# christopher-beckham/gan-heightmaps

Measured on AMD Instinct MI355X. Metric: 512px heightmap+texture train images/sec, higher is better.
Workload: dtype bf16x3; 1 GPU; test1_nobn_bilin_both joint DCGAN+pix2pix train step (train_mode=both), 512x512, batch 4 per GPU, RMSprop lr 1e-4, LSGAN+100*L1; fp32 by operand splitting on the bf16 matrix cores (3 exact bf16 pieces per operand, 6 products, fp32 accumulation); global_batch=4, in_shp=512, parallelism=dp1, hip_graph=False, issue=recorded, streams=3

## Files before the change

### gan_heightmaps_amd/_lib.py

```python
import ctypes as C
import os

_HERE = os.path.dirname(os.path.abspath(__file__))
LIB_PATH = os.path.join(_HERE, "libghm.so")


class GhmError(RuntimeError):
    pass


class ConvDesc(C.Structure):
    _fields_ = [("N", C.c_int32), ("C", C.c_int32), ("H", C.c_int32), ("W", C.c_int32),
                ("K", C.c_int32), ("Ho", C.c_int32), ("Wo", C.c_int32),
                ("kh", C.c_int32), ("kw", C.c_int32), ("stride", C.c_int32), ("pad", C.c_int32),
                ("x_nstride", C.c_int64), ("y_nstride", C.c_int64)]


class RenderParams(C.Structure):
    _fields_ = [("pos", C.c_float * 3), ("yaw", C.c_float), ("pitch", C.c_float), ("fov", C.c_float),
                ("Hi", C.c_int32), ("Wi", C.c_int32),
                ("height_scale", C.c_float), ("step", C.c_float), ("max_dist", C.c_float),
                ("sun_azimuth", C.c_float), ("sun_elevation", C.c_float), ("shadows", C.c_int32),
                ("softness", C.c_float), ("ambient", C.c_float), ("haze", C.c_float),
                ("horizon", C.c_float * 3), ("zenith", C.c_float * 3), ("accel", C.c_int32), ("out_u8", C.c_int32)]
# ... 111 lines not shown
    "ghm_maxpool2_fwd": [_p, _p, _p, _i32, _i32, _i32, _i32],
    "ghm_maxpool2_bwd": [_p, _p, _p, _p, _p, _i32, _i32, _i32, _i32, _i32, _f],
    "ghm_avgpool_fwd": [_p, _p, _p, _i32, _i32, _i32, _i32, _i32],
    "ghm_avgpool_bwd": [_p, _p, _p, _i32, _i32, _i32, _i32, _i32],
    "ghm_dropout": [_p, _p, _i64, _p, _i64, _i32, _i32, _i32, _f, C.c_uint32, _p],
    "ghm_counter_tick": [_p, _p],
    "ghm_transpose_weights_batched": [_p, _p, _i32, _i32],
    "ghm_upconv_collapse_weights": [_p, _p, _p, _p, _p, _i32, _i32],
    "ghm_upconv_collapse_batched": [_p, _p, _i32, _i32],
    "ghm_upconv_expand_batched": [_p, _p, _i32, _i32, _i32],
    "ghm_blconv_frame_sizes": [_i32, _i32, _i32, _i32, _i32, C.POINTER(_i64), C.POINTER(_i64)],
    "ghm_blconv_frame_fwd": [_p, _p, _i64, _p, _p, _i64, _i32, _i32, _i32, _i32, _i32, _p],
    "ghm_blconv_frame_gather": [_p, _p, _i64, _i32, _i32, _i32, _i32, _i32, _p],
    "ghm_blconv_frame_dgrad": [_p, _p, _p, _p, _i64, _i32, _i32, _i32, _i32, _i32],
    "ghm_blconv_frame_wgrad": [_p, _p, _p, _p, _i32, _i32, _i32, _i32, _i32],
    "ghm_blconv_fwd_split": [_p, _D, _p, _i64, _i64, _p, _p, _p, _i32],
    "ghm_blconv_dgrad_split": [_p, _D, _p, _i64, _i64, _p, _p, _i32, _i32],
    "ghm_blconv_wgrad_split": [_p, _D, _p, _i64, _i64, _p, _i64, _i64, _p, _p, _i32, _i32],
    "ghm_upconv_expand_wgrad": [_p, _p, _p, _i32, _i32, _i32],
    "ghm_pp_to_hi": [_p, _p, _p, _i64, _i32, _i32, _i32, _i32],
    "ghm_hi_to_pp": [_p, _p, _i64, _p, _i32, _i32, _i32, _i32],
    "ghm_upsample_nearest2_fwd": [_p, _p, _i64, _p, _i32, _i32, _i32, _i32],
    "ghm_upsample_nearest2_bwd": [_p, _p, _p, _i64, _i32, _i32, _i32, _i32, _i32],
    "ghm_upsample_bilinear2_fwd": [_p, _p, _i64, _p, _i32, _i32, _i32, _i32],
    "ghm_upsample_bilinear2_bwd": [_p, _p, _p, _i64, _i32, _i32, _i32, _i32, _i32],
    "ghm_copy_view": [_p, _p, _i64, _p, _i64, _i32, _i32, _i32, _i32],
    "ghm_scale_samples": [_p, _p, _i64, _i32, _i32, _i32, _p, _i64, _p, _i64],
    "ghm_axpby": [_p, _f, _p, _f, _p, _i64],
    "ghm_image_batch": [_p, _p, _i32, _i32, _i32, _i32, _p, _i32, _p, _i64],
    "ghm_texture_gather": [_p, _p, _i32, _i32, _i32, _i32, _i32, _i32, _i32, _i32, _i32, _i32, _i32, _i32, _i32, _p, _i64],
# ... 25 lines not shown
    "ghm_comm_destroy": [_p],
    "ghm_comm_count": [_p, C.POINTER(_i32)],
    "ghm_allreduce_sum": [_p, _p, _i64],
    "ghm_allreduce_sum_bf16": [_p, _p, _i64, _p],
    "ghm_allreduce_max": [_p, _p, _i64],
    "ghm_reduce_scatter_sum": [_p, _p, _i64],
    "ghm_all_gather": [_p, _p, _i64],
    "ghm_conv2d_variant": [_D, _i32, C.c_char_p, _i32],
}
_SPECIAL = {"ghm_last_error": ([], C.c_char_p), "ghm_bn_workspace": ([_i32], C.c_size_t),
            "ghm_dgrad_t_supported": ([_D], C.c_int), "ghm_lp_supported": ([_D, _i32, _i32], C.c_int),
            "ghm_conv2d_pool_supported": ([_D, _i32, _i32], C.c_int),
            "ghm_dgrad_dact_supported": ([_D, _i32], C.c_int),
            "ghm_blconv_supported": ([_i32, _i32, _i32, _i32, _i32], C.c_int),
            "ghm_blconv_split_supported": ([_D, _i32], C.c_int),
            "ghm_lp_q_direct": ([_D, _i32, _i32], C.c_int),
            "ghm_conv_bn_fused_supported": ([_D, _i32], C.c_int),
            "ghm_conv_bn_fused_supported_f32": ([_D], C.c_int),
            "ghm_lp_wgrad_q_supported": ([_D, _i32], C.c_int),
            "ghm_split_supported": ([_D, _i32], C.c_int),
            "ghm_conv2d_wgrad_pooled_split_supported": ([_D], C.c_int),
            "ghm_split_pool_supported": ([_D, _i32], C.c_int),
            "ghm_split_q_direct": ([_D, _i32], C.c_int),
            "ghm_split_dgrad_dact_supported": ([_D], C.c_int),
            "ghm_render_maxmip_elems": ([_i32, _i32], C.c_int64)}

_lib = None


def load():
# ... 55 lines not shown
```

### gan_heightmaps_amd/csrc/conv_bilinear.hip

```cpp
#include <stdlib.h>
#include <string.h>

#include "common.h"

namespace {

typedef float f32x16 __attribute__((ext_vector_type(16)));

__device__ __forceinline__ int bl_job_line(int job) { return job == 0 ? 0 : (job < 3 ? 1 : (job == 3 ? 2 : 3)); }
__device__ __forceinline__ int bl_job_tap(int job, int t) {
    const int fixed = (job == 0 || job == 3) ? 0 : ((job == 1 || job == 4) ? 2 : 1);
    return job < 3 ? fixed * 3 + t : t * 3 + fixed;
}

struct BlGeo {
    int N, C, K, n1, n2, LP;
};

__global__ __launch_bounds__(256) void bl_lines_kernel(const float* __restrict__ x, long xs, BlGeo g, float* __restrict__ FL,
                                                       float* __restrict__ FLt) {
    const long idx = (long)blockIdx.x * 256 + threadIdx.x;
    const long total = (long)g.N * 4 * g.C * g.LP;
    if (idx >= total) return;
    const int ai = (int)(idx % g.LP);
// ... 66 lines not shown
#pragma unroll 4
    for (int c0 = c_lo + 2 * wave; c0 < c_hi; c0 += 8) {
        const int c = c0 + kg;
        const float* w = wp + (long)c * 9 * g.K + k;
        const float* f = fl + (long)c * g.LP;
        const float a0 = w[(long)t0 * g.K], a1 = w[(long)t1 * g.K], a2 = w[(long)t2 * g.K];
        const float b0 = f[0], b1 = f[1], b2 = f[2];
        acc = bl_mfma(a0, b0, acc);
        acc = bl_mfma(a1, b1, acc);
        acc = bl_mfma(a2, b2, acc);
    }
    float* dst = DL + ((((long)sp * 6 + job) * g.N + n) * g.K + blockIdx.x * 32) * g.LP + blockIdx.y * 32;
    bl_reduce_store(acc, dst, g.LP, 1, smem, 32, 32);
}

__global__ __launch_bounds__(256) void bl_wt_kernel(const float* __restrict__ wp, int C, int K, float* __restrict__ wT) {
    const long idx = (long)blockIdx.x * 256 + threadIdx.x;
    if (idx >= (long)9 * K * C) return;
    const int c = (int)(idx % C);
    const long r = idx / C;
    const int k = (int)(r % K), tap = (int)(r / K);
    wT[idx] = wp[((long)c * 9 + tap) * K + k];
}

__global__ __launch_bounds__(256) void bl_gemm_dgrad_kernel(const float* __restrict__ wT, const float* __restrict__ DYL, BlGeo g,
                                                            int splits, float* __restrict__ dFL, int wp_direct) {
    __shared__ float smem[4 * 32 * 33];
    const int lane = threadIdx.x & 63, wave = threadIdx.x >> 6, li = lane & 31, kg = lane >> 5;
    int z = blockIdx.z;
    const int n = z % g.N;
// ... 17 lines not shown
        const float* w1 = wp_direct ? wT + ((long)c * 9 + bl_job_tap(job, 1)) * g.K : wT + bl_job_tap(job, 1) * KC + c;
        const float* w2 = wp_direct ? wT + ((long)c * 9 + bl_job_tap(job, 2)) * g.K : wT + bl_job_tap(job, 2) * KC + c;
#pragma unroll 4
        for (int k0 = k_lo + 2 * wave; k0 < k_hi; k0 += 8) {
            const int k = k0 + kg;
            const float a0 = w0[k * ks], a1 = w1[k * ks], a2 = w2[k * ks];
            const float* d = dy + (long)k * LD;
            const float b0 = d[0], b1 = d[-1], b2 = d[-2];
            acc = bl_mfma(a0, b0, acc);
            acc = bl_mfma(a1, b1, acc);
            acc = bl_mfma(a2, b2, acc);
        }
    }
    float* dst = dFL + ((((long)sp * g.N + n) * 4 + line) * g.C + blockIdx.x * 32) * g.LP + blockIdx.y * 32;
    bl_reduce_store(acc, dst, g.LP, 1, smem, 32, 32);
}

__global__ __launch_bounds__(256) void bl_gemm_wgrad_kernel(const float* __restrict__ DYLt, const float* __restrict__ FLt, BlGeo g,
                                                            int splits, float* __restrict__ dWp, float* __restrict__ direct) {
    __shared__ float smem[4 * 32 * 33];
    const int lane = threadIdx.x & 63, wave = threadIdx.x >> 6, li = lane & 31, kg = lane >> 5;
    const int tap = blockIdx.z % 9, sp = blockIdx.z / 9;
    const int A = tap / 3, B = tap % 3;
    const int k = blockIdx.x * 32 + li, c = blockIdx.y * 32 + li;
    const int LD = g.LP + 32;
    const int rowjob = A == 0 ? 0 : (A == 2 ? 1 : 2), coljob = B == 0 ? 3 : (B == 2 ? 4 : 5);
    const int rowline = A == 0 ? 0 : 1, colline = B == 0 ? 2 : 3;
    f32x16 acc;
#pragma unroll
    for (int e = 0; e < 16; ++e) acc[e] = 0.f;
// ... 140 lines not shown
    *fl_floats = 2 * ((int64_t)N * 4 * C * LP + 64);
    *dyl_floats = 2 * ((int64_t)6 * N * K * (LP + 32));
    return 0;
}

int ghm_blconv_supported(int32_t N, int32_t C, int32_t K, int32_t n1, int32_t n2) { return bl_ok(N, C, K, n1, n2) ? 1 : 0; }

static int bl_splits(long contraction, long tiles, int num_cu) {
    int s = (int)((4L * num_cu + tiles - 1) / tiles);
    const int smax = (int)(contraction / 256);
    if (s > smax) s = smax;
    if (s > 32) s = 32;
    return s < 1 ? 1 : s;
}

int ghm_blconv_frame_fwd(ghm_ctx* ctx, const float* x, int64_t x_nstride, const float* wp, float* y, int64_t y_nstride, int32_t N,
                         int32_t C, int32_t K, int32_t n1, int32_t n2, float* FL) {
    GHM_CHECK(bl_ok(N, C, K, n1, n2), "ghm_blconv_frame_fwd: geometry not served");
    const BlGeo g{N, C, K, n1, n2, bl_lp(n1, n2)};
    hipLaunchKernelGGL(bl_lines_kernel, dim3(ceil_div((long)N * 4 * C * g.LP, 256)), dim3(256), 0, ctx->stream, x, (long)x_nstride, g, FL,
                       FL + ((long)N * 4 * C * g.LP + 64));
    GHM_LAUNCH_CHECK();
    const int used = (2 * (n1 > n2 ? n1 : n2) + 31) / 32;
    const int splits = bl_splits(3L * C, (long)(K / 32) * used * 6 * N, ctx->num_cu);
    void* ws;
    if (ghm_scratch(ctx, (size_t)splits * 6 * N * K * g.LP * 4, &ws)) return -1;
    hipLaunchKernelGGL(bl_gemm_fwd_kernel, dim3(K / 32, used, splits * 6 * N), dim3(256), 0, ctx->stream, wp, (const float*)FL, g, splits,
                       (float*)ws);
    GHM_LAUNCH_CHECK();
    const long nb = 3L * 2 * n2 + 3L * (2 * n1 - 3);
    hipLaunchKernelGGL(bl_scatter_fwd_kernel, dim3(ceil_div((long)N * K * nb, 256)), dim3(256), 0, ctx->stream, (const float*)ws, g, splits,
                       y, (long)y_nstride);
    GHM_LAUNCH_CHECK();
    return 0;
}

int ghm_blconv_frame_gather(ghm_ctx* ctx, const float* dy, int64_t dy_nstride, int32_t N, int32_t C, int32_t K, int32_t n1, int32_t n2,
                            float* DYL) {
    GHM_CHECK(bl_ok(N, C, K, n1, n2), "ghm_blconv_frame_gather: geometry not served");
    const BlGeo g{N, C, K, n1, n2, bl_lp(n1, n2)};
    hipLaunchKernelGGL(bl_gather_dy_kernel, dim3(ceil_div((long)6 * N * K * (g.LP + 32), 256)), dim3(256), 0, ctx->stream, dy,
                       (long)dy_nstride, g, DYL, DYL + (long)6 * N * K * (g.LP + 32));
    GHM_LAUNCH_CHECK();
    return 0;
}

int ghm_blconv_frame_dgrad(ghm_ctx* ctx, const float* DYL, const float* wp, float* dx, int64_t dx_nstride, int32_t N, int32_t C,
                           int32_t K, int32_t n1, int32_t n2) {
    GHM_CHECK(bl_ok(N, C, K, n1, n2), "ghm_blconv_frame_dgrad: geometry not served");
    const BlGeo g{N, C, K, n1, n2, bl_lp(n1, n2)};
    const int used = (2 * (n1 > n2 ? n1 : n2) + 2 + 31) / 32;
    const int splits = bl_splits(6L * K, (long)(C / 32) * used * 4 * N, ctx->num_cu);
    void* ws;
    const size_t part_bytes = (size_t)splits * N * 4 * C * g.LP * 4;
    if (ghm_scratch(ctx, part_bytes + (size_t)9 * K * C * 4, &ws)) return -1;
    float* const wT = (float*)((char*)ws + part_bytes);
    const int direct = GHM_OPT("GHM_BLCONV_NO_WT") ? 1 : 0;
    if (!direct) {
        hipLaunchKernelGGL(bl_wt_kernel, dim3(ceil_div((long)9 * K * C, 256)), dim3(256), 0, ctx->stream, wp, C, K, wT);
        GHM_LAUNCH_CHECK();
    }
    hipLaunchKernelGGL(bl_gemm_dgrad_kernel, dim3(C / 32, used, splits * 4 * N), dim3(256), 0, ctx->stream,
                       direct ? wp : (const float*)wT, DYL, g, splits, (float*)ws, direct);
    GHM_LAUNCH_CHECK();
    const long nb = (long)(n1 >= 2 ? 2 : 1) * n2 + (long)(n2 >= 2 ? 2 : 1) * (n1 > 2 ? n1 - 2 : 0);
    hipLaunchKernelGGL(bl_fold_kernel, dim3(ceil_div((long)N * C * nb, 256)), dim3(256), 0, ctx->stream, (const float*)ws, g, splits, dx,
                       (long)dx_nstride);
// ... 13 lines not shown
                           DYL + (long)6 * N * K * (g.LP + 32), FL + ((long)N * 4 * C * g.LP + 64), g, 1, (float*)nullptr, dwp);
        GHM_LAUNCH_CHECK();
        return 0;
    }
    void* ws;
    if (ghm_scratch(ctx, (size_t)splits * 9 * C * K * 4, &ws)) return -1;
    hipLaunchKernelGGL(bl_gemm_wgrad_kernel, dim3(K / 32, C / 32, splits * 9), dim3(256), 0, ctx->stream,
                       DYL + (long)6 * N * K * (g.LP + 32), FL + ((long)N * 4 * C * g.LP + 64), g, splits, (float*)ws, (float*)nullptr);
    GHM_LAUNCH_CHECK();
    hipLaunchKernelGGL(bl_wgrad_add_kernel, dim3(ceil_div((long)C * 9 * K, 256)), dim3(256), 0, ctx->stream, (const float*)ws, C, K, splits,
                       dwp);
    GHM_LAUNCH_CHECK();
    return 0;
}

}
```

### gan_heightmaps_amd/csrc/elementwise.hip

```cpp
#include "common.h"

namespace {

struct View {
    int N, C, HW;
};

template <int VEC>
__device__ __forceinline__ bool decode(const View v, long& n, long& c, long& i) {
    const long per_row = v.HW / VEC;
    const long idx = (long)blockIdx.x * blockDim.x + threadIdx.x;
    const long total = (long)v.N * v.C * per_row;
    if (idx >= total) return false;
    const long row = idx / per_row;
    i = (idx - row * per_row) * VEC;
    n = row / v.C;
    c = row - n * v.C;
    return true;
}

inline bool aligned16(const void* p) { return ((uintptr_t)p & 15) == 0; }

inline int grid_for(const View v, int vec) { return ceil_div((long)v.N * v.C * (v.HW / vec), 256); }

// ... 745 lines not shown
    float v = 0.f;
#pragma unroll
    for (int pq = 0; pq < 4; ++pq) {
        const int rs = upconv_group(pq >> 1, a) * 3 + upconv_group(pq & 1, b);
        v += dwpc[(((long)c * 9 + rs) * 4 + pq) * K + k];
    }
    dwp5[i] = accumulate ? dwp5[i] + v : v;
}

struct CollapseItem {
    const float* wp5;
    const float* bias;
    float* wpc;
    float* bias4;
    int C, K, block_begin, mode;
};

__device__ __forceinline__ float blconv_coef(int p, int r, int a) {
    if (p == 0) return r == 1 ? (a == 1 ? 1.f : 0.5f) : ((r == 0 && a == 0) || (r == 2 && a == 2) ? 0.5f : 0.f);
    return r == 0 ? 0.f : (a == 1 ? 0.5f : ((r == 1 && a == 0) || (r == 2 && a == 2) ? 1.f : 0.f));
}

__global__ __launch_bounds__(256) void upconv_collapse_batched_kernel(const CollapseItem* __restrict__ items, int n) {
    int li = 0;
    for (int i = 1; i < n; ++i)
        if ((int)blockIdx.x >= items[i].block_begin) li = i;
    const CollapseItem it = items[li];
    const long total = (long)it.C * 36 * it.K;
    const long i = (long)(blockIdx.x - it.block_begin) * 256 + threadIdx.x;
    if (i < total) {
        const int K = it.K;
        const int k = (int)(i % K);
        long t = i / K;
        const int pq = (int)(t % 4); t /= 4;
        const int rs = (int)(t % 9);
        const int c = (int)(t / 9);
        const int p = pq >> 1, q = pq & 1, r = rs / 3, s_ = rs % 3;
        float v = 0.f;
        if (it.mode == 1) {
            for (int a = 0; a < 3; ++a)
                for (int b = 0; b < 3; ++b) {
                    const float cf = blconv_coef(p, r, a) * blconv_coef(q, s_, b);
                    if (cf != 0.f) v += cf * it.wp5[((long)c * 9 + a * 3 + b) * K + k];
                }
// ... 762 lines not shown
```

### gan_heightmaps_amd/device.py

```python
import ctypes as C

import numpy as np

from . import _lib
from ._lib import ConvDesc, call

ACT_CODES = {'linear': 0, 'relu': 1, 'lrelu': 2, 'sigmoid': 3, 'tanh': 4}
DTYPE_CODES = {'f32': 0, 'bf16': 1, 'f16': 2}
SPLIT = 'bf16x3'
DTYPE_CODES[SPLIT] = 3
SPLIT2 = 'bf16x2'
DTYPE_CODES[SPLIT2] = 4
SPLITS = {SPLIT: 3, SPLIT2: 2}


def device_count():
    n = C.c_int32(0)
    call("ghm_device_count", C.byref(n))
    return n.value


class DevTensor:
    __slots__ = ("dev", "ptr", "shape", "nstride", "base")

# ... 376 lines not shown
        call("ghm_conv2d_fwd", self.h, C.byref(d), _vp(x), _vp(wp), _vp(bias), _vp(y), ACT_CODES[act], alpha,
             int(accumulate))

    def conv2d_dgrad(self, d, dy, wp, dx, bias=None, act='linear', alpha=0.0, accumulate=False):
        call("ghm_conv2d_dgrad", self.h, C.byref(d), _vp(dy), _vp(wp), _vp(bias), _vp(dx), ACT_CODES[act], alpha,
             int(accumulate))

    def dgrad_t_supported(self, d):
        return bool(_lib.load().ghm_dgrad_t_supported(C.byref(d)))

    def transpose_weights(self, d, wp, wpT):
        call("ghm_conv2d_transpose_weights", self.h, C.byref(d), _vp(wp), _vp(wpT))

    def collapse_table(self, items):
        rec = np.zeros(len(items), dtype=[('wp5', '<u8'), ('bias', '<u8'), ('wpc', '<u8'), ('b4', '<u8'), ('C', '<i4'),
                                          ('K', '<i4'), ('b0', '<i4'), ('pad', '<i4')])
        b0 = 0
        for i, (w5, b, wpc, b4, Cc, K, *mode) in enumerate(items):
            rec[i] = (w5.ptr, b.ptr if b is not None else 0, wpc.ptr, b4.ptr if b4 is not None else 0, Cc, K, b0, mode[0] if mode else 0)
            b0 += (36 * Cc * K + 4 * K + 255) // 256
        ptr = self.dev.alloc(max(rec.nbytes, 40))
        self.dev.h2d(ptr, rec.view(np.uint8))
        return ptr, len(items), b0

    def upconv_collapse_batched(self, table):
        ptr, n, blocks = table
        call("ghm_upconv_collapse_batched", self.h, C.c_void_p(ptr), n, blocks)

    def expand_table(self, items):
        rec = np.zeros(len(items), dtype=[('dwpc', '<u8'), ('dwp5', '<u8'), ('C', '<i4'), ('K', '<i4'), ('b0', '<i4'),
                                          ('pad', '<i4')])
        b0 = 0
        for i, (dwpc, dwp5, Cc, K, *mode) in enumerate(items):
            rec[i] = (dwpc.ptr, dwp5.ptr, Cc, K, b0, mode[0] if mode else 0)
            b0 += (25 * Cc * K + 255) // 256
        ptr = self.dev.alloc(max(rec.nbytes, 32))
# ... 11 lines not shown
        a, b = C.c_int64(), C.c_int64()
        call("ghm_blconv_frame_sizes", int(N), int(Cc), int(K), int(n1), int(n2), C.byref(a), C.byref(b))
        return a.value, b.value

    def blconv_frame_fwd(self, x, wp, y_pp, K, FL):
        call("ghm_blconv_frame_fwd", self.h, _vp(x), x.nstride, _vp(wp), _vp(y_pp), y_pp.nstride, x.N, x.Cc, int(K), x.H, x.W, _vp(FL))

    def blconv_frame_gather(self, dy_pp, Cc, K, DYL):
        call("ghm_blconv_frame_gather", self.h, _vp(dy_pp), dy_pp.nstride, dy_pp.N, int(Cc), int(K), dy_pp.H, dy_pp.W, _vp(DYL))

    def blconv_frame_dgrad(self, DYL, wp, dx, K):
        call("ghm_blconv_frame_dgrad", self.h, _vp(DYL), _vp(wp), _vp(dx), dx.nstride, dx.N, dx.Cc, int(K), dx.H, dx.W)

    def blconv_frame_wgrad(self, DYL, FL, dwp, N, Cc, K, n1, n2):
        call("ghm_blconv_frame_wgrad", self.h, _vp(DYL), _vp(FL), _vp(dwp), int(N), int(Cc), int(K), int(n1), int(n2))

    def blconv_split_supported(self, d, kind, dtype):
        return dtype in SPLITS and bool(_lib.load().ghm_blconv_split_supported(C.byref(d), int(kind)))

    def blconv_fwd_split(self, d, xq, wq, bias, y, dtype):
        call("ghm_blconv_fwd_split", self.h, C.byref(d), C.c_void_p(xq.ptr), xq.nstride, xq.pstride, _vp(wq), _vp(bias), _vp(y),
             SPLITS[dtype])

    def blconv_dgrad_split(self, d, dyq, wqT, dx, dtype, accumulate=False):
        call("ghm_blconv_dgrad_split", self.h, C.byref(d), C.c_void_p(dyq.ptr), dyq.nstride, dyq.pstride, _vp(wqT), _vp(dx),
             int(accumulate), SPLITS[dtype])

    def blconv_wgrad_split(self, d, xq, dyq, dwp, ws, dtype, accumulate=False):
        call("ghm_blconv_wgrad_split", self.h, C.byref(d), C.c_void_p(xq.ptr), xq.nstride, xq.pstride, C.c_void_p(dyq.ptr),
             dyq.nstride, dyq.pstride, _vp(dwp), _vp(ws), int(accumulate), SPLITS[dtype])
# ... 602 lines not shown
```

### gan_heightmaps_amd/engine.py

```python
import os

import numpy as np

from . import layers as L
from .architectures.layers import BilinearUpsample2DLayer
from .device import SPLITS, DevTensor, QTensor, conv_desc, pack_conv_w, unpack_conv_w
from .nonlinearities import linear

ALIGN = 64
FWD, DGRAD, WGRAD, DGRAD_T = 0, 1, 2, 3


def _align(n):
    return (n + ALIGN - 1) // ALIGN * ALIGN


class ParamStore:

    def __init__(self, dev, params, pad_to=1):
        self.dev = dev
        self.params = list(params)
        nt = ns = 0
        for p in self.params:
            n = int(np.prod(p.shape))
# ... 256 lines not shown

class NetPlan:

    def __init__(self, dev, ops, out_layer, batch, store, inputs=None, out_tensor=None, name="net", side=None,
                 bn_groups=1, rng_seed=0, rng_counter=None, dtype='f32'):
        self.dev, self.ops, self.batch, self.store, self.name = dev, ops, batch, store, name
        self.side = side
        assert dtype in ('f32', 'bf16', 'f16') or dtype in SPLITS, dtype
        self.dtype = dtype
        self.bn_groups = bn_groups
        nodes, of = _build_ir(out_layer)
        self.out_node = _rewrite(of[id(out_layer)], dtype)
        self.order = _toposort(self.out_node)
        self.node_of_layer = of
        self.input_nodes = [n for n in self.order if n.op == 'input']
        self._shapes()
        self._fuse_convpool()
        self._place(inputs or {}, out_tensor)
        self.use_q = self.dtype != 'f32' and os.environ.get("GHM_NO_Q") is None and hasattr(ops, 'q_pack')
        self.q_epi = self.use_q
        for n in self.order:
            n.outq = None
        if self.use_q:
            self._place_q()
        self._scratch = {}
        self._collapse_tab = None
        self._last_grads = {}
        self.bn_ws = None
        cmax = max([n.shape[1] for n in self.order if n.op == 'bn'] + [0])
        if cmax:
# ... 131 lines not shown
                    n.aux['mean_g'] = [n.aux['mean'], self.dev.empty((1, C, 1, 1))]
                    n.aux['inv_g'] = [n.aux['inv'], self.dev.empty((1, C, 1, 1))]
            if n.op == 'convpool':
                n.aux['mask'] = self.dev.alloc(int(np.prod(n.shape)))
            if n.op == 'upconv':
                C, K = n.inputs[0].shape[1], n.shape[1]
                for name in ('wpc', 'wpcT', 'dwpc'):
                    n.aux[name] = self.dev.empty((1, C * 9 * 4 * K, 1, 1))
                n.aux['b4'] = self.dev.empty((1, 4 * K, 1, 1))
                if n.attrs.get('mode') == 1:
                    xs = n.inputs[0].shape
                    if not self.ops.blconv_supported(xs[0], C, K, xs[2], xs[3]):
                        raise NotImplementedError("bilinear up-sample convolution %r: geometry not served by the library" % (n,))
                    nfl, ndyl = self.ops.blconv_frame_sizes(xs[0], C, K, xs[2], xs[3])
                    n.aux['fl'], n.aux['dyl'] = self.dev.empty((1, nfl, 1, 1)), self.dev.empty((1, ndyl, 1, 1))

    def _place_q(self):
        need = []
        for n in self.order:
            if n.op in ('conv', 'convpool'):
                d = self._desc(n, n.inputs[0].out, self._full(n))
            elif n.op == 'upconv':
                d = self._upconv_desc(n, n.inputs[0].out)
            else:
                continue
            if self._lp(d, FWD) and n.inputs[0].shape[1] % 8 == 0 and self._q_viewable(n.inputs[0]):
                need.append(n.inputs[0])

        def get_outq(n):
            if n.outq is not None:
# ... 151 lines not shown
        if b > self._wgrad_ws_bytes:
            if self.wgrad_ws is not None:
                self.dev.free(self.wgrad_ws)
            self.wgrad_ws = self.dev.alloc(b)
            self._wgrad_ws_bytes = b

    def emit_forward(self, prog, deterministic=False, update_running=True, lp_done=None):
        ops, st = self.ops, self.store
        if self.dropout_nodes and not deterministic:
            prog.append(("rng_tick", lambda c=self.rng_counter: ops.counter_tick(c)))
        ups = [n for n in self.order if n.op == 'upconv']
        if ups:
            if self._collapse_tab is None:
                self._collapse_tab = ops.collapse_table(
                    [(st.value(n.layer.W), st.value(n.layer.b), n.aux['wpc'], n.aux['b4'], n.inputs[0].shape[1], n.shape[1],
                      n.attrs.get('mode', 0)) for n in ups])
            prog.append(("collapse_w", lambda t=self._collapse_tab: ops.upconv_collapse_batched(t)))
        if self._lp_table is not None:
            prog.append(("lp_pack", lambda t=self._lp_table: ops.lp_pack_batched(t, self.dtype)))
        ctx = _ForwardCtx(prog, deterministic, update_running, lp_done)
        for n in self.order:
            if id(n) in ctx.fused_bn:
                continue
            lower = getattr(self, '_fwd_' + n.op, None)
            if lower is None:
                raise NotImplementedError(n.op)
            q_direct = lower(ctx, n)
            if n.outq is not None and not q_direct:
                self._q_pack(prog, n.out, n.outq)

    def _q_pack(self, prog, t, q):
# ... 165 lines not shown
        w5 = st.value(n.layer.W)
        wpc, b4, K = n.aux['wpc'], n.aux['b4'], n.shape[1]
        bl = n.attrs.get('mode') == 1
        label = ('blconv' if bl else 'upconv') + "_fwd"
        y4 = y.reshape((x.N, 4 * K, x.H, x.W))
        wq = None
        if self._lp(d, FWD):
            wq = self._lp_pack_entry(prog, d, wpc, ('c', id(n.layer.W)), False, None)
        if wq is not None and xq is not None and self._bl_skip(n, d, FWD) and a == linear:
            prog.append((label, lambda: ops.blconv_fwd_split(d, xq, wq, b4, y4, self.dtype), bl_meta(conv_meta(ops, d, FWD, self.dtype))))
        else:
            prog.append(self._conv_fwd_entry(label, d, x, xq, wpc, wq, b4, y4, None, a))
        if bl:
            if a != linear:
                raise NotImplementedError("bilinear up-sample convolution with its own nonlinearity")
            prog.append(("blconv_frame_fwd", lambda fl=n.aux['fl']: ops.blconv_frame_fwd(x, w5, y4, K, fl)))
        return False

    def _fwd_pp_to_hi(self, ctx, n):
        ops, x, y, yq = self.ops, n.inputs[0].out, n.out, n.outq
        if id(n) in ctx.fused_hi:
            return self.q_epi
        if yq is not None and self.q_epi and y.nstride % 2 == 0:
            y32 = y if self._fp32_needed(n) else None
            ctx.prog.append(("pp_to_hi", lambda: ops.pp_to_hi_q(x, y32, yq)))
            return True
        ctx.prog.append(("pp_to_hi", lambda: ops.pp_to_hi(x, y)))
        return False

    def _fwd_dropout(self, ctx, n):
        ops, x, y = self.ops, n.inputs[0].out, n.out
# ... 453 lines not shown
            if G4q is not None and plan._bl_skip(n, d, DGRAD):
                prog.append((label, lambda: ops.blconv_dgrad_split(d, G4q, wqT, gi, plan.dtype, acc),
                             bl_meta(conv_meta(ops, d, DGRAD_T, dt))))
            elif G4q is not None:
                prog.append((label, lambda: ops.conv2d_dgrad_lp_q(d, G4q, wqT, gi, None, plan.dtype, None, 'linear', 0.0, acc),
                             conv_meta(ops, d, DGRAD_T, dt)))
            else:
                prog.append((label, lambda: ops.conv2d_dgrad_lp(d, G4, wqT, gi, plan.dtype, None, 'linear', 0.0, acc),
                             conv_meta(ops, d, DGRAD_T, dt)))
        elif C > 4 and ops.dgrad_t_supported(d):
            self.transpose_once(('c', id(l.W)), d, wpc, wpcT)
            prog.append((label, lambda: ops.conv2d_dgrad_t(d, G4, wpcT, gi, None, 'linear', 0.0, acc), conv_meta(ops, d, DGRAD_T)))
        else:
            prog.append((label, lambda: ops.conv2d_dgrad(d, G4, wpc, gi, None, 'linear', 0.0, acc), conv_meta(ops, d, DGRAD)))
        if bl:
            prog.append(("blconv_frame_dgrad", lambda dyl=n.aux['dyl'], w3=self.st.value(l.W): ops.blconv_frame_dgrad(dyl, w3, gi, K)))

    def bwd_dropout(self, n, G, xin, x, y, need_dx):
        if need_dx:
            gi, acc = self.target(xin)
            if acc or self.nslice is not None:
                raise NotImplementedError("DropoutLayer input with several consumers / sample slices")
            ops = self.ops
            self.prog.append(("dropout_bwd", lambda p=n.attrs['p'], k=n.aux['key'], c=self.plan.rng_counter: ops.dropout(G, gi, p, k, c)))
            self.mark_written(xin)

    def bwd_pp_to_hi(self, n, G, xin, x, y, need_dx):
        if need_dx and self.nslice is None and self.plan._bn_hi(xin) and G.nstride % 2 == 0:
            self.grads[id(xin)] = G
            self.hi_grads.add(id(xin))
            self.mark_written(xin)
# ... 189 lines not shown
```

### include/ghm.h

```cpp
#ifndef GHM_H
#define GHM_H

#include <stddef.h>
#include <stdint.h>

#ifdef __cplusplus
extern "C" {
#endif

typedef struct ghm_ctx ghm_ctx;
typedef struct ghm_graph ghm_graph;
typedef struct ghm_step ghm_step;

enum { GHM_DTYPE_F32 = 0, GHM_DTYPE_BF16 = 1, GHM_DTYPE_F16 = 2 };

enum { GHM_ACT_LINEAR = 0, GHM_ACT_RELU = 1, GHM_ACT_LRELU = 2, GHM_ACT_SIGMOID = 3, GHM_ACT_TANH = 4 };

typedef struct {
    int32_t N;
    int32_t C, H, W;
    int32_t K, Ho, Wo;
    int32_t kh, kw, stride, pad;
    int64_t x_nstride;
    int64_t y_nstride;
// ... 192 lines not shown
int ghm_counter_tick(ghm_ctx* ctx, void* counter);
int ghm_upconv_collapse_weights(ghm_ctx* ctx, const float* wp5, const float* bias, float* wpc, float* bias4, int32_t C, int32_t K);
int ghm_upconv_collapse_batched(ghm_ctx* ctx, const void* table, int32_t n_items, int32_t total_blocks);
int ghm_upconv_expand_wgrad(ghm_ctx* ctx, const float* dwpc, float* dwp5, int32_t C, int32_t K, int32_t accumulate);
int ghm_upconv_expand_batched(ghm_ctx* ctx, const void* table, int32_t n_items, int32_t total_blocks, int32_t accumulate);
int ghm_blconv_supported(int32_t N, int32_t C, int32_t K, int32_t n1, int32_t n2);
int ghm_blconv_frame_sizes(int32_t N, int32_t C, int32_t K, int32_t n1, int32_t n2, int64_t* fl_floats, int64_t* dyl_floats);
int ghm_blconv_frame_fwd(ghm_ctx* ctx, const float* x, int64_t x_nstride, const float* wp, float* y_pp, int64_t y_nstride, int32_t N,
                         int32_t C, int32_t K, int32_t n1, int32_t n2, float* FL);
int ghm_blconv_frame_gather(ghm_ctx* ctx, const float* dy_pp, int64_t dy_nstride, int32_t N, int32_t C, int32_t K, int32_t n1,
                            int32_t n2, float* DYL);
int ghm_blconv_frame_dgrad(ghm_ctx* ctx, const float* DYL, const float* wp, float* dx, int64_t dx_nstride, int32_t N, int32_t C,
                           int32_t K, int32_t n1, int32_t n2);
int ghm_blconv_frame_wgrad(ghm_ctx* ctx, const float* DYL, const float* FL, float* dwp, int32_t N, int32_t C, int32_t K, int32_t n1,
                           int32_t n2);
int ghm_blconv_split_supported(const ghm_conv_desc* d, int32_t kind);
int ghm_blconv_fwd_split(ghm_ctx* ctx, const ghm_conv_desc* d, const void* xq, int64_t xq_nstride, int64_t xq_pstride, const void* wq,
                         const float* bias, float* y, int32_t pieces);
int ghm_blconv_dgrad_split(ghm_ctx* ctx, const ghm_conv_desc* d, const void* dyq, int64_t dyq_nstride, int64_t dyq_pstride,
                           const void* wqT, float* dx, int32_t accumulate, int32_t pieces);
int ghm_blconv_wgrad_split(ghm_ctx* ctx, const ghm_conv_desc* d, const void* xq, int64_t xq_nstride, int64_t xq_pstride,
                           const void* dyq, int64_t dyq_nstride, int64_t dyq_pstride, float* dwp, void* workspace,
                           int32_t accumulate, int32_t pieces);
int ghm_pp_to_hi(ghm_ctx* ctx, const float* pp, float* hi, int64_t hi_nstride, int32_t N, int32_t K, int32_t H, int32_t W);
int ghm_hi_to_pp(ghm_ctx* ctx, const float* hi, int64_t hi_nstride, float* pp, int32_t N, int32_t K, int32_t H, int32_t W);
int ghm_upsample_bilinear2_fwd(ghm_ctx* ctx, const float* x, int64_t x_nstride, float* y, int32_t N, int32_t C, int32_t H, int32_t W);
int ghm_upsample_bilinear2_bwd(ghm_ctx* ctx, const float* dy, float* dx, int64_t dx_nstride, int32_t N, int32_t C, int32_t H, int32_t W, int32_t accumulate);
int ghm_copy_view(ghm_ctx* ctx, const float* x, int64_t x_nstride, float* y, int64_t y_nstride, int32_t N, int32_t C, int32_t HW, int32_t accumulate);
int ghm_scale_samples(ghm_ctx* ctx, float* x, int64_t x_nstride, int32_t N, int32_t C, int32_t HW, const float* num, int64_t num_nstride,
                      const float* den, int64_t den_nstride);
// ... 132 lines not shown
```

Measured before the change: 323.0 images/s.

## Batch samples per block in bilinear frame GEMMs and precompute transposed weights

Adds templated forward and dgrad frame GEMM kernels in which each block handles up to four samples, so every weight load is reused across the batch instead of being reloaded per sample. The split count is recomputed for the smaller grid. The dgrad path now takes a transposed weight copy that is built inside the existing batched weight-collapse launch, replacing a separate per-call transpose. The trade-off is more accumulator registers per thread (NB f32x16 accumulators), which may lower occupancy, plus an extra weight buffer per bilinear layer.

Measured after the change: 323.1 images/s (median of 5 runs). No clear change (+0.0%).

```diff
diff --git a/gan_heightmaps_amd/_lib.py b/gan_heightmaps_amd/_lib.py
--- a/gan_heightmaps_amd/_lib.py
+++ b/gan_heightmaps_amd/_lib.py
@@ -149,6 +149,8 @@
     "ghm_blconv_frame_gather": [_p, _p, _i64, _i32, _i32, _i32, _i32, _i32, _p],
     "ghm_blconv_frame_dgrad": [_p, _p, _p, _p, _i64, _i32, _i32, _i32, _i32, _i32],
     "ghm_blconv_frame_wgrad": [_p, _p, _p, _p, _i32, _i32, _i32, _i32, _i32],
+    "ghm_blconv_frame_fwd_batched": [_p, _p, _i64, _p, _p, _i64, _i32, _i32, _i32, _i32, _i32, _p],
+    "ghm_blconv_frame_dgrad_batched": [_p, _p, _p, _p, _i64, _i32, _i32, _i32, _i32, _i32],
     "ghm_blconv_fwd_split": [_p, _D, _p, _i64, _i64, _p, _p, _p, _i32],
     "ghm_blconv_dgrad_split": [_p, _D, _p, _i64, _i64, _p, _p, _i32, _i32],
     "ghm_blconv_wgrad_split": [_p, _D, _p, _i64, _i64, _p, _i64, _i64, _p, _p, _i32, _i32],
@@ -204,6 +206,7 @@
             "ghm_dgrad_dact_supported": ([_D, _i32], C.c_int),
             "ghm_blconv_supported": ([_i32, _i32, _i32, _i32, _i32], C.c_int),
             "ghm_blconv_split_supported": ([_D, _i32], C.c_int),
+            "ghm_blconv_frame_splits": ([_p, _i32, _i32, _i32, _i32, _i32, _i32, _i32], C.c_int),
             "ghm_lp_q_direct": ([_D, _i32, _i32], C.c_int),
             "ghm_conv_bn_fused_supported": ([_D, _i32], C.c_int),
             "ghm_conv_bn_fused_supported_f32": ([_D], C.c_int),
diff --git a/gan_heightmaps_amd/csrc/conv_bilinear.hip b/gan_heightmaps_amd/csrc/conv_bilinear.hip
--- a/gan_heightmaps_amd/csrc/conv_bilinear.hip
+++ b/gan_heightmaps_amd/csrc/conv_bilinear.hip
@@ -104,6 +104,53 @@
     bl_reduce_store(acc, dst, g.LP, 1, smem, 32, 32);
 }
 
+template <int NB>
+__global__ __launch_bounds__(256) void bl_gemm_fwd_nb_kernel(const float* __restrict__ wp, const float* __restrict__ FL, BlGeo g,
+                                                             int splits, float* __restrict__ DL) {
+    __shared__ float smem[4 * 32 * 33];
+    const int lane = threadIdx.x & 63, wave = threadIdx.x >> 6, li = lane & 31, kg = lane >> 5;
+    const int groups = (g.N + NB - 1) / NB;
+    int z = blockIdx.z;
+    const int n0 = (z % groups) * NB;
+    z /= groups;
+    const int job = z % 6, sp = z / 6;
+    const int k = blockIdx.x * 32 + li, pos = blockIdx.y * 32 + li;
+    const int per = ((g.C / 2 + splits - 1) / splits) * 2;
+    const int c_lo = sp * per, c_hi = min(g.C, c_lo + per);
+    const long sample = (long)4 * g.C * g.LP;
+    const float* fl[NB];
+#pragma unroll
+    for (int s = 0; s < NB; ++s) fl[s] = FL + min(n0 + s, g.N - 1) * sample + ((long)bl_job_line(job) * g.C) * g.LP + pos;
+    const int t0 = bl_job_tap(job, 0), t1 = bl_job_tap(job, 1), t2 = bl_job_tap(job, 2);
+    f32x16 acc[NB];
+#pragma unroll
+    for (int s = 0; s < NB; ++s)
+#pragma unroll
+        for (int e = 0; e < 16; ++e) acc[s][e] = 0.f;
+#pragma unroll 2
+    for (int c0 = c_lo + 2 * wave; c0 < c_hi; c0 += 8) {
+        const int c = c0 + kg;
+        const float* w = wp + (long)c * 9 * g.K + k;
+        const float a0 = w[(long)t0 * g.K], a1 = w[(long)t1 * g.K], a2 = w[(long)t2 * g.K];
+#pragma unroll
+        for (int s = 0; s < NB; ++s) {
+            const float* f = fl[s] + (long)c * g.LP;
+            const float b0 = f[0], b1 = f[1], b2 = f[2];
+            acc[s] = bl_mfma(a0, b0, acc[s]);
+            acc[s] = bl_mfma(a1, b1, acc[s]);
+            acc[s] = bl_mfma(a2, b2, acc[s]);
+        }
+    }
+#pragma unroll
+    for (int s = 0; s < NB; ++s) {
+        if (n0 + s < g.N) {
+            float* dst = DL + ((((long)sp * 6 + job) * g.N + n0 + s) * g.K + blockIdx.x * 32) * g.LP + blockIdx.y * 32;
+            bl_reduce_store(acc[s], dst, g.LP, 1, smem, 32, 32);
+        }
+        __syncthreads();
+    }
+}
+
 __global__ __launch_bounds__(256) void bl_wt_kernel(const float* __restrict__ wp, int C, int K, float* __restrict__ wT) {
     const long idx = (long)blockIdx.x * 256 + threadIdx.x;
     if (idx >= (long)9 * K * C) return;
@@ -151,6 +198,60 @@
     }
     float* dst = dFL + ((((long)sp * g.N + n) * 4 + line) * g.C + blockIdx.x * 32) * g.LP + blockIdx.y * 32;
     bl_reduce_store(acc, dst, g.LP, 1, smem, 32, 32);
+}
+
+template <int NB>
+__global__ __launch_bounds__(256) void bl_gemm_dgrad_nb_kernel(const float* __restrict__ wT, const float* __restrict__ DYL, BlGeo g,
+                                                               int splits, float* __restrict__ dFL) {
+    __shared__ float smem[4 * 32 * 33];
+    const int lane = threadIdx.x & 63, wave = threadIdx.x >> 6, li = lane & 31, kg = lane >> 5;
+    const int groups = (g.N + NB - 1) / NB;
+    int z = blockIdx.z;
+    const int n0 = (z % groups) * NB;
+    z /= groups;
+    const int line = z % 4, sp = z / 4;
+    const int c = blockIdx.x * 32 + li, ai = blockIdx.y * 32 + li;
+    const int per = ((g.K / 2 + splits - 1) / splits) * 2;
+    const int k_lo = sp * per, k_hi = min(g.K, k_lo + per);
+    const int LD = g.LP + 32;
+    f32x16 acc[NB];
+#pragma unroll
+    for (int s = 0; s < NB; ++s)
+#pragma unroll
+        for (int e = 0; e < 16; ++e) acc[s][e] = 0.f;
+    const int job_lo = line == 0 ? 0 : (line == 1 ? 1 : (line == 2 ? 3 : 4));
+    const int njobs = (line == 0 || line == 2) ? 1 : 2;
+    const long KC = (long)g.K * g.C;
+    for (int jj = 0; jj < njobs; ++jj) {
+        const int job = job_lo + jj;
+        const float* dy[NB];
+#pragma unroll
+        for (int s = 0; s < NB; ++s) dy[s] = DYL + (((long)job * g.N + min(n0 + s, g.N - 1)) * g.K) * LD + ai + 2;
+        const float* w0 = wT + bl_job_tap(job, 0) * KC + c;
+        const float* w1 = wT + bl_job_tap(job, 1) * KC + c;
+        const float* w2 = wT + bl_job_tap(job, 2) * KC + c;
+#pragma unroll 2
+        for (int k0 = k_lo + 2 * wave; k0 < k_hi; k0 += 8) {
+            const int k = k0 + kg;
+            const float a0 = w0[(long)k * g.C], a1 = w1[(long)k * g.C], a2 = w2[(long)k * g.C];
+#pragma unroll
+            for (int s = 0; s < NB; ++s) {
+                const float* d = dy[s] + (long)k * LD;
+                const float b0 = d[0], b1 = d[-1], b2 = d[-2];
+                acc[s] = bl_mfma(a0, b0, acc[s]);
+                acc[s] = bl_mfma(a1, b1, acc[s]);
+                acc[s] = bl_mfma(a2, b2, acc[s]);
+            }
+        }
+    }
+#pragma unroll
+    for (int s = 0; s < NB; ++s) {
+        if (n0 + s < g.N) {
+            float* dst = dFL + ((((long)sp * g.N + n0 + s) * 4 + line) * g.C + blockIdx.x * 32) * g.LP + blockIdx.y * 32;
+            bl_reduce_store(acc[s], dst, g.LP, 1, smem, 32, 32);
+        }
+        __syncthreads();
+    }
 }
 
 __global__ __launch_bounds__(256) void bl_gemm_wgrad_kernel(const float* __restrict__ DYLt, const float* __restrict__ FLt, BlGeo g,
@@ -321,6 +422,16 @@
     return s < 1 ? 1 : s;
 }
 
+static int bl_nb(int N) { return N >= 4 ? 4 : (N >= 2 ? 2 : 1); }
+static int bl_fwd_used(int n1, int n2) { return (2 * (n1 > n2 ? n1 : n2) + 31) / 32; }
+static int bl_dgrad_used(int n1, int n2) { return (2 * (n1 > n2 ? n1 : n2) + 2 + 31) / 32; }
+static int bl_fwd_splits(int N, int C, int K, int n1, int n2, int nb, int num_cu) {
+    return bl_splits(3L * C, (long)(K / 32) * bl_fwd_used(n1, n2) * 6 * ((N + nb - 1) / nb), num_cu);
+}
+static int bl_dgrad_splits(int N, int C, int K, int n1, int n2, int nb, int num_cu) {
+    return bl_splits(6L * K, (long)(C / 32) * bl_dgrad_used(n1, n2) * 4 * ((N + nb - 1) / nb), num_cu);
+}
+
 int ghm_blconv_frame_fwd(ghm_ctx* ctx, const float* x, int64_t x_nstride, const float* wp, float* y, int64_t y_nstride, int32_t N,
                          int32_t C, int32_t K, int32_t n1, int32_t n2, float* FL) {
     GHM_CHECK(bl_ok(N, C, K, n1, n2), "ghm_blconv_frame_fwd: geometry not served");
@@ -328,8 +439,8 @@
     hipLaunchKernelGGL(bl_lines_kernel, dim3(ceil_div((long)N * 4 * C * g.LP, 256)), dim3(256), 0, ctx->stream, x, (long)x_nstride, g, FL,
                        FL + ((long)N * 4 * C * g.LP + 64));
     GHM_LAUNCH_CHECK();
-    const int used = (2 * (n1 > n2 ? n1 : n2) + 31) / 32;
-    const int splits = bl_splits(3L * C, (long)(K / 32) * used * 6 * N, ctx->num_cu);
+    const int used = bl_fwd_used(n1, n2);
+    const int splits = bl_fwd_splits(N, C, K, n1, n2, 1, ctx->num_cu);
     void* ws;
     if (ghm_scratch(ctx, (size_t)splits * 6 * N * K * g.LP * 4, &ws)) return -1;
     hipLaunchKernelGGL(bl_gemm_fwd_kernel, dim3(K / 32, used, splits * 6 * N), dim3(256), 0, ctx->stream, wp, (const float*)FL, g, splits,
@@ -356,8 +467,8 @@
                            int32_t K, int32_t n1, int32_t n2) {
     GHM_CHECK(bl_ok(N, C, K, n1, n2), "ghm_blconv_frame_dgrad: geometry not served");
     const BlGeo g{N, C, K, n1, n2, bl_lp(n1, n2)};
-    const int used = (2 * (n1 > n2 ? n1 : n2) + 2 + 31) / 32;
-    const int splits = bl_splits(6L * K, (long)(C / 32) * used * 4 * N, ctx->num_cu);
+    const int used = bl_dgrad_used(n1, n2);
+    const int splits = bl_dgrad_splits(N, C, K, n1, n2, 1, ctx->num_cu);
     void* ws;
     const size_t part_bytes = (size_t)splits * N * 4 * C * g.LP * 4;
     if (ghm_scratch(ctx, part_bytes + (size_t)9 * K * C * 4, &ws)) return -1;
@@ -401,4 +512,63 @@
     return 0;
 }
 
-}
+int ghm_blconv_frame_splits(ghm_ctx* ctx, int32_t kind, int32_t batched, int32_t N, int32_t C, int32_t K, int32_t n1, int32_t n2) {
+    if (!bl_ok(N, C, K, n1, n2)) return 0;
+    const int nb = batched ? bl_nb(N) : 1;
+    if (kind == 0) return bl_fwd_splits(N, C, K, n1, n2, nb, ctx->num_cu);
+    if (kind == 1) return bl_dgrad_splits(N, C, K, n1, n2, nb, ctx->num_cu);
+    const int npmin = n1 < n2 ? n1 : n2;
+    int splits = bl_splits((long)2 * N * (n1 + n2), (long)(K / 32) * (C / 32) * 9, ctx->num_cu);
+    if (splits > npmin / 4) splits = npmin / 4 > 0 ? npmin / 4 : 1;
+    return splits;
+}
+
+int ghm_blconv_frame_fwd_batched(ghm_ctx* ctx, const float* x, int64_t x_nstride, const float* wp, float* y, int64_t y_nstride,
+                                 int32_t N, int32_t C, int32_t K, int32_t n1, int32_t n2, float* FL) {
+    GHM_CHECK(bl_ok(N, C, K, n1, n2), "ghm_blconv_frame_fwd_batched: geometry not served");
+    const BlGeo g{N, C, K, n1, n2, bl_lp(n1, n2)};
+    hipLaunchKernelGGL(bl_lines_kernel, dim3(ceil_div((long)N * 4 * C * g.LP, 256)), dim3(256), 0, ctx->stream, x, (long)x_nstride, g, FL,
+                       FL + ((long)N * 4 * C * g.LP + 64));
+    GHM_LAUNCH_CHECK();
+    const int used = bl_fwd_used(n1, n2), nb = bl_nb(N);
+    const int splits = bl_fwd_splits(N, C, K, n1, n2, nb, ctx->num_cu);
+    void* ws;
+    if (ghm_scratch(ctx, (size_t)splits * 6 * N * K * g.LP * 4, &ws)) return -1;
+    const dim3 grid(K / 32, used, splits * 6 * ((N + nb - 1) / nb));
+#define BL_FWD_NB(NB) hipLaunchKernelGGL((bl_gemm_fwd_nb_kernel<NB>), grid, dim3(256), 0, ctx->stream, wp, (const float*)FL, g, splits, (float*)ws)
+    if (nb == 4) BL_FWD_NB(4);
+    else if (nb == 2) BL_FWD_NB(2);
+    else BL_FWD_NB(1);
+#undef BL_FWD_NB
+    GHM_LAUNCH_CHECK();
+    const long nbp = 3L * 2 * n2 + 3L * (2 * n1 - 3);
+    hipLaunchKernelGGL(bl_scatter_fwd_kernel, dim3(ceil_div((long)N * K * nbp, 256)), dim3(256), 0, ctx->stream, (const float*)ws, g, splits,
+                       y, (long)y_nstride);
+    GHM_LAUNCH_CHECK();
+    return 0;
+}
+
+int ghm_blconv_frame_dgrad_batched(ghm_ctx* ctx, const float* DYL, const float* wT, float* dx, int64_t dx_nstride, int32_t N,
+                                   int32_t C, int32_t K, int32_t n1, int32_t n2) {
+    GHM_CHECK(bl_ok(N, C, K, n1, n2), "ghm_blconv_frame_dgrad_batched: geometry not served");
+    GHM_CHECK(wT != nullptr, "ghm_blconv_frame_dgrad_batched: no transposed weights");
+    const BlGeo g{N, C, K, n1, n2, bl_lp(n1, n2)};
+    const int used = bl_dgrad_used(n1, n2), nb = bl_nb(N);
+    const int splits = bl_dgrad_splits(N, C, K, n1, n2, nb, ctx->num_cu);
+    void* ws;
+    if (ghm_scratch(ctx, (size_t)splits * N * 4 * C * g.LP * 4, &ws)) return -1;
+    const dim3 grid(C / 32, used, splits * 4 * ((N + nb - 1) / nb));
+#define BL_DGRAD_NB(NB) hipLaunchKernelGGL((bl_gemm_dgrad_nb_kernel<NB>), grid, dim3(256), 0, ctx->stream, wT, DYL, g, splits, (float*)ws)
+    if (nb == 4) BL_DGRAD_NB(4);
+    else if (nb == 2) BL_DGRAD_NB(2);
+    else BL_DGRAD_NB(1);
+#undef BL_DGRAD_NB
+    GHM_LAUNCH_CHECK();
+    const long nbp = (long)(n1 >= 2 ? 2 : 1) * n2 + (long)(n2 >= 2 ? 2 : 1) * (n1 > 2 ? n1 - 2 : 0);
+    hipLaunchKernelGGL(bl_fold_kernel, dim3(ceil_div((long)N * C * nbp, 256)), dim3(256), 0, ctx->stream, (const float*)ws, g, splits, dx,
+                       (long)dx_nstride);
+    GHM_LAUNCH_CHECK();
+    return 0;
+}
+
+}
diff --git a/gan_heightmaps_amd/csrc/elementwise.hip b/gan_heightmaps_amd/csrc/elementwise.hip
--- a/gan_heightmaps_amd/csrc/elementwise.hip
+++ b/gan_heightmaps_amd/csrc/elementwise.hip
@@ -783,6 +783,7 @@
     float* wpc;
     float* bias4;
     int C, K, block_begin, mode;
+    float* wT;
 };
 
 __device__ __forceinline__ float blconv_coef(int p, int r, int a) {
@@ -797,6 +798,19 @@
     const CollapseItem it = items[li];
     const long total = (long)it.C * 36 * it.K;
     const long i = (long)(blockIdx.x - it.block_begin) * 256 + threadIdx.x;
+    const int own = (int)((total + 4L * it.K + 255) / 256);
+    if (it.wT && (int)(blockIdx.x - it.block_begin) >= own) {
+        __shared__ float tile[32][33];
+        int tb = blockIdx.x - it.block_begin - own;
+        const int kt = tb % (it.K / 32); tb /= it.K / 32;
+        const int ct = tb % (it.C / 32), tap = tb / (it.C / 32);
+        if (tap >= 9) return;
+        const int lx = threadIdx.x & 31, ly = threadIdx.x >> 5;
+        for (int r = ly; r < 32; r += 8) tile[r][lx] = it.wp5[((long)(ct * 32 + r) * 9 + tap) * it.K + kt * 32 + lx];
+        __syncthreads();
+        for (int r = ly; r < 32; r += 8) it.wT[((long)tap * it.K + kt * 32 + r) * it.C + ct * 32 + lx] = tile[lx][r];
+        return;
+    }
     if (i < total) {
         const int K = it.K;
         const int k = (int)(i % K);
diff --git a/gan_heightmaps_amd/device.py b/gan_heightmaps_amd/device.py
--- a/gan_heightmaps_amd/device.py
+++ b/gan_heightmaps_amd/device.py
@@ -414,12 +414,19 @@
 
     def collapse_table(self, items):
         rec = np.zeros(len(items), dtype=[('wp5', '<u8'), ('bias', '<u8'), ('wpc', '<u8'), ('b4', '<u8'), ('C', '<i4'),
-                                          ('K', '<i4'), ('b0', '<i4'), ('pad', '<i4')])
+                                          ('K', '<i4'), ('b0', '<i4'), ('pad', '<i4'), ('wT', '<u8')])
         b0 = 0
-        for i, (w5, b, wpc, b4, Cc, K, *mode) in enumerate(items):
-            rec[i] = (w5.ptr, b.ptr if b is not None else 0, wpc.ptr, b4.ptr if b4 is not None else 0, Cc, K, b0, mode[0] if mode else 0)
+        for i, (w5, b, wpc, b4, Cc, K, *more) in enumerate(items):
+            mode = more[0] if more else 0
+            wT = more[1] if len(more) > 1 else None
+            if wT is not None and (mode != 1 or Cc % 32 or K % 32):
+                raise ValueError("collapse_table: transposed weights need the bilinear form with C and K multiples of 32")
+            rec[i] = (w5.ptr, b.ptr if b is not None else 0, wpc.ptr, b4.ptr if b4 is not None else 0, Cc, K, b0, mode,
+                      wT.ptr if wT is not None else 0)
             b0 += (36 * Cc * K + 4 * K + 255) // 256
-        ptr = self.dev.alloc(max(rec.nbytes, 40))
+            if wT is not None:
+                b0 += 9 * (Cc // 32) * (K // 32)
+        ptr = self.dev.alloc(max(rec.nbytes, 56))
         self.dev.h2d(ptr, rec.view(np.uint8))
         return ptr, len(items), b0
 
@@ -461,6 +468,16 @@
 
     def blconv_frame_wgrad(self, DYL, FL, dwp, N, Cc, K, n1, n2):
         call("ghm_blconv_frame_wgrad", self.h, _vp(DYL), _vp(FL), _vp(dwp), int(N), int(Cc), int(K), int(n1), int(n2))
+
+    def blconv_frame_splits(self, kind, batched, N, Cc, K, n1, n2):
+        return int(_lib.load().ghm_blconv_frame_splits(self.h, int(kind), int(bool(batched)), int(N), int(Cc), int(K), int(n1), int(n2)))
+
+    def blconv_frame_fwd_batched(self, x, wp, y_pp, K, FL):
+        call("ghm_blconv_frame_fwd_batched", self.h, _vp(x), x.nstride, _vp(wp), _vp(y_pp), y_pp.nstride, x.N, x.Cc, int(K), x.H, x.W,
+             _vp(FL))
+
+    def blconv_frame_dgrad_batched(self, DYL, wT, dx, K):
+        call("ghm_blconv_frame_dgrad_batched", self.h, _vp(DYL), _vp(wT), _vp(dx), dx.nstride, dx.N, dx.Cc, int(K), dx.H, dx.W)
 
     def blconv_split_supported(self, d, kind, dtype):
         return dtype in SPLITS and bool(_lib.load().ghm_blconv_split_supported(C.byref(d), int(kind)))
diff --git a/gan_heightmaps_amd/engine.py b/gan_heightmaps_amd/engine.py
--- a/gan_heightmaps_amd/engine.py
+++ b/gan_heightmaps_amd/engine.py
@@ -294,6 +294,8 @@
         self.order = _toposort(self.out_node)
         self.node_of_layer = of
         self.input_nodes = [n for n in self.order if n.op == 'input']
+        self.bl_frame_old = os.environ.get("GHM_BLCONV_FRAME_OLD") is not None
+        self.bl_frame_wt = not self.bl_frame_old and os.environ.get("GHM_BLCONV_NO_WT") is None
         self._shapes()
         self._fuse_convpool()
         self._place(inputs or {}, out_tensor)
@@ -455,6 +457,8 @@
                         raise NotImplementedError("bilinear up-sample convolution %r: geometry not served by the library" % (n,))
                     nfl, ndyl = self.ops.blconv_frame_sizes(xs[0], C, K, xs[2], xs[3])
                     n.aux['fl'], n.aux['dyl'] = self.dev.empty((1, nfl, 1, 1)), self.dev.empty((1, ndyl, 1, 1))
+                    if self.bl_frame_wt:
+                        n.aux['wT'] = self.dev.empty((1, 9 * C * K, 1, 1))
 
     def _place_q(self):
         need = []
@@ -636,7 +640,7 @@
             if self._collapse_tab is None:
                 self._collapse_tab = ops.collapse_table(
                     [(st.value(n.layer.W), st.value(n.layer.b), n.aux['wpc'], n.aux['b4'], n.inputs[0].shape[1], n.shape[1],
-                      n.attrs.get('mode', 0)) for n in ups])
+                      n.attrs.get('mode', 0), n.aux.get('wT')) for n in ups])
             prog.append(("collapse_w", lambda t=self._collapse_tab: ops.upconv_collapse_batched(t)))
         if self._lp_table is not None:
             prog.append(("lp_pack", lambda t=self._lp_table: ops.lp_pack_batched(t, self.dtype)))
@@ -832,7 +836,8 @@
         if bl:
             if a != linear:
                 raise NotImplementedError("bilinear up-sample convolution with its own nonlinearity")
-            prog.append(("blconv_frame_fwd", lambda fl=n.aux['fl']: ops.blconv_frame_fwd(x, w5, y4, K, fl)))
+            frame_fwd = ops.blconv_frame_fwd if self.bl_frame_old else ops.blconv_frame_fwd_batched
+            prog.append(("blconv_frame_fwd", lambda fl=n.aux['fl']: frame_fwd(x, w5, y4, K, fl)))
         return False
 
     def _fwd_pp_to_hi(self, ctx, n):
@@ -1316,7 +1321,10 @@
         else:
             prog.append((label, lambda: ops.conv2d_dgrad(d, G4, wpc, gi, None, 'linear', 0.0, acc), conv_meta(ops, d, DGRAD)))
         if bl:
-            prog.append(("blconv_frame_dgrad", lambda dyl=n.aux['dyl'], w3=self.st.value(l.W): ops.blconv_frame_dgrad(dyl, w3, gi, K)))
+            if 'wT' in n.aux:
+                prog.append(("blconv_frame_dgrad", lambda dyl=n.aux['dyl'], wT=n.aux['wT']: ops.blconv_frame_dgrad_batched(dyl, wT, gi, K)))
+            else:
+                prog.append(("blconv_frame_dgrad", lambda dyl=n.aux['dyl'], w3=self.st.value(l.W): ops.blconv_frame_dgrad(dyl, w3, gi, K)))
 
     def bwd_dropout(self, n, G, xin, x, y, need_dx):
         if need_dx:
diff --git a/include/ghm.h b/include/ghm.h
--- a/include/ghm.h
+++ b/include/ghm.h
@@ -230,6 +230,11 @@
                            int32_t K, int32_t n1, int32_t n2);
 int ghm_blconv_frame_wgrad(ghm_ctx* ctx, const float* DYL, const float* FL, float* dwp, int32_t N, int32_t C, int32_t K, int32_t n1,
                            int32_t n2);
+int ghm_blconv_frame_splits(ghm_ctx* ctx, int32_t kind, int32_t batched, int32_t N, int32_t C, int32_t K, int32_t n1, int32_t n2);
+int ghm_blconv_frame_fwd_batched(ghm_ctx* ctx, const float* x, int64_t x_nstride, const float* wp, float* y_pp, int64_t y_nstride,
+                                 int32_t N, int32_t C, int32_t K, int32_t n1, int32_t n2, float* FL);
+int ghm_blconv_frame_dgrad_batched(ghm_ctx* ctx, const float* DYL, const float* wT, float* dx, int64_t dx_nstride, int32_t N,
+                                   int32_t C, int32_t K, int32_t n1, int32_t n2);
 int ghm_blconv_split_supported(const ghm_conv_desc* d, int32_t kind);
 int ghm_blconv_fwd_split(ghm_ctx* ctx, const ghm_conv_desc* d, const void* xq, int64_t xq_nstride, int64_t xq_pstride, const void* wq,
                          const float* bias, float* y, int32_t pieces);
```
